# JoelTankard/web-rwkv-gguf

Measured on AMD Instinct MI355X. Metric: tokens/sec RWKV-7 1.5B Q4_K_M decode @1 GPU; achieved HBM GB/s vs roofline, higher is better.
Workload: dtype f16; 1 GPU; RWKV-7 World 1.5B Q4_K_M (Q4_K matrices, Q6_K head, F16 LoRA) batch=1 greedy decode, fused kernels under hipGraph; decode_engine=on, streams_per_gpu=1, pipelines_per_gpu=1, streams=1, parallelism=single

## Files before the change

web-rwkv-gguf_amd/csrc/wrk_v7.hip:

```cpp
#include "wrk_internal.h"
#include "wrk_v7.h"
#include "wrk_v7_engine.h"

#define LOCK(ctx) std::lock_guard<std::recursive_mutex> _lk((ctx)->mu)

static constexpr float LN_EPS = 1.0e-5f;
static constexpr float GN_EPS = 64.0e-5f;
static constexpr float L2_EPS = 1.0e-12f;

using wrk::mat_job;

int32_t wrk_v7_model::ensure_scratch(uint32_t T, uint32_t NH) {
    if (T <= scratch_tokens && NH <= scratch_headers && scratch) return WRK_OK;
    if (ctx->capturing_here()) return wrk_fail(ctx, WRK_E_ARG, "scratch must be sized before capture");
    const uint32_t nt = T > scratch_tokens ? T : scratch_tokens;
    const uint32_t nh = NH > scratch_headers ? NH : scratch_headers;
    WRK_HIP(ctx, hipStreamSynchronize(ctx->stream));
    drop_graphs();
    if (scratch) hipFree(scratch);
    scratch = nullptr;
    const size_t D = d.num_emb, F = d.num_hidden, V = d.num_vocab;
    size_t off = 0;
    auto take = [&](size_t bytes) { size_t o = off; off += wrk_up256(bytes); return o; };
    const size_t esz = act_dtype == WRK_F32 ? 4 : 2;
// ... 449 lines not shown
                     const uint32_t* cursors, uint32_t T, const uint32_t* headers, uint32_t NH, const uint32_t* targets, float* logprob,
                     uint32_t* rank, uint32_t mode) {
    return v7_job(ctx, m, st, {tokens, emb_rows, cursors, T, headers, NH, nullptr, nullptr, true, targets, logprob, rank}, mode);
}

int32_t wrk_v7_model_set_frame_dtype(wrk_ctx* ctx, wrk_v7_model* m, uint32_t dtype) {
    if (!ctx || !m) return WRK_E_ARG;
    LOCK(ctx);
    WRK_ARG(ctx, dtype == WRK_F16 || dtype == WRK_F32, "frame dtype must be WRK_F16 or WRK_F32");
    WRK_ARG(ctx, !ctx->capturing_here(), "cannot change the frame inside a capture");
    if (dtype == m->act_dtype) return WRK_OK;
    WRK_HIP(ctx, hipSetDevice(ctx->device));
    WRK_HIP(ctx, hipStreamSynchronize(ctx->stream));
    m->drop_graphs();
    if (m->scratch) hipFree(m->scratch);
    m->scratch = nullptr;
    m->scratch_tokens = m->scratch_headers = 0;
    m->act_dtype = dtype;
    for (hipStream_t ls : m->lane_streams) WRK_HIP(ctx, hipStreamSynchronize(ls));
    std::vector<wrk_v7_model*> old_lanes;
    old_lanes.swap(m->lanes);
    for (wrk_v7_model* lane : old_lanes) wrk_v7_model_destroy(lane);
    return WRK_OK;
}

int32_t wrk_v7_model_engine_status(wrk_ctx* ctx, wrk_v7_model* m, char* why, size_t capacity) {
    if (!ctx || !m) return WRK_E_ARG;
    LOCK(ctx);
    WRK_HIP(ctx, hipSetDevice(ctx->device));
    WRK_ARG(ctx, !ctx->capturing_here(), "not inside a capture");
    const int32_t rc = m->ensure_engine();
    if (rc != WRK_OK) return rc;
    if (why && capacity) {
        const std::string& w = m->engine ? std::string() : (m->engine_tried ? m->engine_why : std::string("disabled (WRK_ENGINE=0 or f32 frames)"));
        snprintf(why, capacity, "%s", w.c_str());
    }
    return m->engine ? 1 : 0;
}

int32_t wrk_v7_infer_layer(wrk_ctx* ctx, wrk_v7_model* m, wrk_v7_state* st, uint32_t layer, const void* x, const void* v_first,
                           const uint32_t* cursors, uint32_t T, uint32_t mode) {
    if (!ctx || !m || !st || !x || !cursors) return WRK_E_ARG;
    LOCK(ctx);
    WRK_HIP(ctx, hipSetDevice(ctx->device));
    WRK_ARG(ctx, !ctx->capturing_here(), "wrk_v7_infer_layer cannot be captured");
    WRK_ARG(ctx, layer < m->d.num_layer, "layer %u out of range", layer);
    WRK_ARG(ctx, T >= 1, "no tokens");
    WRK_ARG(ctx, layer == 0 || v_first, "layers above 0 read the layer-0 value (att_v0)");
    WRK_ARG(ctx, st->num_emb == m->d.num_emb && st->num_layer == m->d.num_layer, "state does not belong to this model");
    wrk_job_shape sh;
    int32_t rc = wrk_job_check(ctx, st, cursors, T, nullptr, 0, nullptr, 0, &sh);
    if (rc == WRK_OK) rc = m->ensure_scratch(T, 1);
    if (rc == WRK_OK && T == 1 && mode == 1) rc = m->ensure_engine();
    if (rc != WRK_OK) return rc;
    const size_t esz = m->act_dtype == WRK_F32 ? 4 : 2;
    rc = wrk_buf_write_raw(ctx, m->s.cursors, cursors, (size_t)T * 4);
    if (rc == WRK_OK) rc = wrk_buf_write_raw(ctx, m->s.x, x, (size_t)T * m->d.num_emb * esz);
    if (rc == WRK_OK && v_first) rc = wrk_buf_write_raw(ctx, m->s.att_v0, v_first, (size_t)T * m->d.num_emb * esz);
    if (rc != WRK_OK) return rc;
    m->layer_begin = layer; m->layer_end = layer + 1; m->skip_embed = true;
    m->wkv_nseq = sh.nseq;
    { const char* ei = getenv("WRK_ENGINE_INSPECT"); m->engine_skip_once = !(ei && ei[0] == '1'); }
    if (mode == 1 && sh.one_token_each && sh.nseq == T && m->act_dtype == WRK_F16) rc = m->enqueue_fused_decode(st, T, 0, true, false, false, false, cursors[0] & 0xff, sh.contiguous);
    else rc = m->enqueue_ops(st, T, 0, true, mode == 1);
    m->layer_begin = 0; m->layer_end = 0xffffffffu; m->skip_embed = false; m->engine_skip_once = false;
    if (rc != WRK_OK) return rc;
    WRK_LAUNCH_CHECK(ctx);
// ... 147 lines not shown
```

web-rwkv-gguf_amd/csrc/wrk_v7_engine.h:

```cpp
#pragma once
#include <stdint.h>

#include "wrk_internal.h"

namespace wrk {

constexpr int ENG_K1_JOBS = 7;
constexpr uint32_t ENG_NO_HEAD = 0xffffffffu;

struct EngJob {
    uint32_t rows, row_bytes, f16;
    uint32_t act, mix;
    uint32_t wg0, nwg, rows_per_wg;
    uint32_t gbase;
    uint32_t headed;
};

struct EngShape {
    uint32_t D, F, H, nwg;
    uint32_t rw, ra, rg, rv;
    uint32_t rb_d, rb_f;
    uint32_t rb_w2, rb_a2, rb_g2, rb_v2;
    EngJob k1[ENG_K1_JOBS];
    uint32_t k3_rpw, k5_rpw, k6_rpw;
// ... 2 lines not shown
    float ln_eps, gn_eps, l2_eps;
    uint32_t layer_begin, layer_end, rescale;
    uint32_t batch, state_rows;
    uint32_t x_from_granules;
};

struct EngLayer {
    const uint8_t *w_r, *w_k, *w_v, *w1, *a1, *g1, *v1;
    const uint8_t *w2, *a2, *g2, *v2;
    const uint8_t *w_o, *ffn_k, *ffn_v;
};
enum { ENG_V_LN1W, ENG_V_LN1B, ENG_V_LN2W, ENG_V_LN2B, ENG_V_MIX0, ENG_V_W0 = ENG_V_MIX0 + 6, ENG_V_A0, ENG_V_V0, ENG_V_RK, ENG_V_KK, ENG_V_KA,
       ENG_V_GNW, ENG_V_GNB, ENG_V_FFNXK, ENG_NV };
enum { ENG_S_O = ENG_K1_JOBS, ENG_S_FK, ENG_S_FV, ENG_NS = 16 };

struct EngArgs {
    EngShape S;
    const EngLayer* layers;
    const void* vecs;
    const float* scal;
    unsigned long long* gran;
    const void* x_in;
    const uint32_t* x_row;
    void* x_out;
    void* v_first;
    float* state;
    uint32_t num_batch;
    uint32_t* fail;
    unsigned long long* stamps;
    uint32_t stamp_layer;
};
constexpr int ENG_STAMPS = 32;

}

struct wrk_v7_model;
struct wrk_v7_state;
struct wrk_v7_engine;
int32_t wrk_v7_engine_create(wrk_v7_model* m, wrk_v7_engine** out);
void wrk_v7_engine_destroy(wrk_v7_engine* e);
int32_t wrk_v7_engine_enqueue(wrk_v7_engine* e, hipStream_t q, wrk_v7_state* st, uint32_t batch, uint32_t l0, uint32_t l1, const void* x_in,
                              void* x_out, void* v_first, const uint32_t* token = nullptr);
bool wrk_v7_engine_has_table(const wrk_v7_engine* e);
int32_t wrk_v7_engine_check(wrk_v7_engine* e);
void wrk_v7_engine_report(wrk_v7_engine* e);
```

web-rwkv-gguf_amd/csrc/wrk_v7_engine.hip:

```cpp
#include "wrk_device.h"
#include "wrk_v7.h"
#include "wrk_dmv_body.h"
#include "wrk_v7_engine.h"
#include "wrk_lora_dev.h"

#include <algorithm>
#include <string>

namespace wrk {

#define ENG_LDS __attribute__((address_space(3)))
typedef ENG_LDS unsigned char lds_u8;

#define ENG_BAR() asm volatile("s_waitcnt lgkmcnt(0)\n\ts_barrier" ::: "memory")

constexpr uint32_t ENG_SPIN_MAX = 1u << 21;

__device__ __forceinline__ uint32_t eng_tag(uint32_t layer, uint32_t stage) { return layer * 8u + stage + 1u; }

__device__ __forceinline__ void eng_store_granule(unsigned long long* g, uint32_t tag, uint32_t payload) {
    __hip_atomic_store(g, ((unsigned long long)tag << 32) | payload, __ATOMIC_RELAXED, __HIP_MEMORY_SCOPE_AGENT);
}
__device__ __forceinline__ uint32_t pack_h2(float a, float b) {
    const f16x2 h = {(f16)a, (f16)b};
// ... 137 lines not shown
}

struct EngFin {
    uint32_t act;
    float scale;
    const ENG_LDS f16* res;
    float post;
};
__device__ __forceinline__ float eng_finish(const EngFin& f, uint32_t row, float v) {
    float o = act_apply(f.act, v * f.scale);
    if (f.res) o = r16(o) + (float)f.res[row];
    return o;
}

template <int KIND, bool R16, int XI, int RB, class GIDX>
__device__ __forceinline__ void eng_rows(const lds_u8* slot, uint32_t row_bytes, uint32_t K, const ENG_LDS f16* xs, uint32_t row0, uint32_t r_begin,
                                         uint32_t r_end, const EngFin& fin, ENG_LDS uint32_t* pub, unsigned long long* gran, uint32_t tag, GIDX gidx,
                                         uint32_t lane) {
    if (r_begin >= r_end) return;
    const uint32_t kpad = (K + 15u) & ~15u;
    const uint32_t nch = num_chunks<KIND>(K, kpad);
    XRegs x[1][XI];
#pragma unroll
    for (int ci = 0; ci < XI; ++ci) {
        const uint32_t c = lane + 64u * ci;
        x[0][ci] = lds_x<KIND>(xs, min(c, nch - 1));
        if (c >= nch) {
            const f16x8 z = {0, 0, 0, 0, 0, 0, 0, 0};
            x[0][ci].v[0] = x[0][ci].v[1] = x[0][ci].v[2] = x[0][ci].v[3] = z;
        }
        x_sums<KIND>(x[0][ci]);
    }
    static_assert(RB == 2 || RB == 4, "rows per batch");
    for (uint32_t ri = r_begin; ri < r_end; ri += RB) {
        Raw raw[RB][XI];
#pragma unroll
        for (int rb = 0; rb < RB; ++rb) {
            const lds_u8* rowp = slot + (size_t)min(ri + rb, r_end - 1) * row_bytes;
#pragma unroll
            for (int ci = 0; ci < XI; ++ci) raw[rb][ci] = lds_raw<KIND>(rowp, K, min(lane + 64u * ci, nch - 1));
        }
        float v[4] = {0.0f, 0.0f, 0.0f, 0.0f};
#pragma unroll
        for (int rb = 0; rb < RB; ++rb) {
            float acc[1] = {0.0f};
#pragma unroll
            for (int ci = 0; ci < XI; ++ci) dot_raw_tokens<KIND, R16, 1, XI>(raw[rb][ci], min(lane + 64u * ci, nch - 1), x, ci, acc);
            v[rb] = wave_sum(acc[0]);
        }
        if (lane < RB / 2) {
            const uint32_t ra = ri + 2 * lane;
            if (ra < r_end) {
                const float o0 = eng_finish(fin, row0 + ra, lane ? v[2] : v[0]) * fin.post;
                const float o1 = eng_finish(fin, row0 + ra + 1, lane ? v[3] : v[1]) * fin.post;
                if (pub) pub[ra >> 1] = pack_h2(o0, o1);
                else eng_store_granule(gran + gidx(row0 + ra), tag, pack_h2(o0, o1));
            }
        }
    }
}

template <class GIDX>
__device__ __forceinline__ void eng_publish(const ENG_LDS uint32_t* pub, uint32_t nrows, uint32_t row0, unsigned long long* gran, uint32_t tag, GIDX gidx,
                                            uint32_t lane) {
    for (uint32_t i = lane; 2 * i < nrows; i += 64) eng_store_granule(gran + gidx(row0 + 2 * i), tag, pub[i]);
}

template <int VPT>
__device__ __forceinline__ void eng_ln_mix(bool active, const ENG_LDS f16* xraw, ENG_LDS f16* xs, ENG_LDS f16* ln_out, ENG_LDS float* red, uint32_t K, float eps,
                                           const f16x8 (&wv)[VPT], const f16x8 (&bv)[VPT], const f16x8 (&mv)[VPT], const f32x4 (&pv)[VPT][2],
                                           uint32_t tid, uint32_t lane, uint32_t wave) {
    const uint32_t nvec = K >> 3;
    f16x8 xv[VPT];
    float c0 = 0.0f;
    if (active) {
#pragma unroll
        for (int v = 0; v < VPT; ++v) xv[v] = *(const ENG_LDS f16x8*)(xraw + min(tid + 256u * v, nvec - 1) * 8);
        c0 = (float)xraw[0];
        float s1 = 0.0f, s2 = 0.0f;
#pragma unroll
        for (int v = 0; v < VPT; ++v)
            if (tid + 256u * v < nvec)
#pragma unroll
                for (int e = 0; e < 8; ++e) { const float dl = (float)xv[v][e] - c0; s1 += dl; s2 = __builtin_fmaf(dl, dl, s2); }
        s1 = wave_sum(s1);
        s2 = wave_sum(s2);
        if (lane == 0) { red[wave] = s1; red[4 + wave] = s2; }
    }
    ENG_BAR();
    if (active) {
        const float a1 = (red[0] + red[1]) + (red[2] + red[3]);
        const float a2 = (red[4] + red[5]) + (red[6] + red[7]);
        const float md = a1 / (float)K;
        const float mean = c0 + md;
        const float dev = 1.0f / sqrtf(fmaxf(a2 / (float)K - md * md, 0.0f) + eps);
#pragma unroll
        for (int v = 0; v < VPT; ++v) {
            const uint32_t i = tid + 256u * v;
            if (i >= nvec) continue;
            f16x8 yv, o;
#pragma unroll
            for (int e = 0; e < 8; ++e) {
                yv[e] = (f16)__builtin_fmaf(((float)xv[v][e] - mean) * dev, (float)wv[v][e], (float)bv[v][e]);
                o[e] = (f16)wgsl_mix((float)yv[e], pv[v][e >> 2][e & 3], (float)mv[v][e]);
            }
            *(ENG_LDS f16x8*)(xs + i * 8) = o;
            *(ENG_LDS f16x8*)(ln_out + i * 8) = yv;
        }
    }
    ENG_BAR();
}

constexpr int ENG_K2_BARRIERS = 6;
template <int XD, bool R16, int QK, int NCW>
__global__ void __launch_bounds__((NCW + 2) * 64) v7_engine_kernel(const EngArgs A, const uint32_t* __restrict__ wg_head) {
    extern __shared__ __attribute__((aligned(16))) unsigned char eng_smem_generic[];
    lds_u8* smem = (lds_u8*)eng_smem_generic;
    const EngShape& S = A.S;
    const uint32_t tid_all = threadIdx.x;
    const uint32_t wave = (uint32_t)__builtin_amdgcn_readfirstlane((int)(tid_all >> 6));
    const uint32_t wg = blockIdx.x;
    const uint32_t D = S.D, F = S.F;
    const uint32_t head = wg_head[2 * wg], k1r = wg_head[2 * wg + 1];
    const bool is_head = head != ENG_NO_HEAD;
    ENG_LDS uint32_t* abort_flag = (ENG_LDS uint32_t*)(smem + S.lds_misc + 1008);
    ENG_LDS float* red = (ENG_LDS float*)(smem + S.lds_misc);
    ENG_LDS float* part = (ENG_LDS float*)(smem + S.lds_misc + 64);
    ENG_LDS uint32_t* pub = (ENG_LDS uint32_t*)(smem + S.lds_misc + 64);
    ENG_LDS f16* xraw0 = (ENG_LDS f16*)(smem + S.lds_xraw0);
    ENG_LDS f16* xraw1 = (ENG_LDS f16*)(smem + S.lds_xraw1);
    ENG_LDS f16* xs = (ENG_LDS f16*)(smem + S.lds_xs);
    ENG_LDS f16* lnbuf = (ENG_LDS f16*)(smem + S.lds_ln);
    ENG_LDS f16* auxbuf = (ENG_LDS f16*)(smem + S.lds_xs + D * 2u);
    const uint32_t naux = S.rw + S.ra + S.rg + S.rv;
    ENG_LDS float* k2f = (ENG_LDS float*)(smem + S.lds_xs + D * 2u + ((naux + 192u) * 2u + 15u & ~15u));

    uint32_t j1 = ENG_K1_JOBS;
#pragma unroll
    for (int j = 0; j < ENG_K1_JOBS; ++j)
        if (k1r >= S.k1[j].wg0 && k1r < S.k1[j].wg0 + S.k1[j].nwg) j1 = j;
    const uint32_t k1_row0 = j1 < ENG_K1_JOBS ? (k1r - S.k1[j1].wg0) * S.k1[j1].rows_per_wg : 0u;
    const uint32_t k1_rows = j1 < ENG_K1_JOBS ? min(S.k1[j1].rows_per_wg, S.k1[j1].rows - k1_row0) : 0u;
    const uint32_t k1_rb = j1 < ENG_K1_JOBS ? S.k1[j1].row_bytes : 0u;
    const uint32_t k3_row0 = wg * S.k3_rpw, k3_rows = k3_row0 < D ? min(S.k3_rpw, D - k3_row0) : 0u;
    const uint32_t k5_row0 = wg * S.k5_rpw, k5_rows = k5_row0 < F ? min(S.k5_rpw, F - k5_row0) : 0u;
    const uint32_t k6_row0 = wg * S.k6_rpw, k6_rows = k6_row0 < D ? min(S.k6_rpw, D - k6_row0) : 0u;
    const uint32_t srows = S.state_rows;
    auto layer_state = [&](uint32_t l) { return A.state + ((size_t)l * A.num_batch + S.batch) * srows * D; };
    auto k1_src = [&](const EngLayer& L) -> const uint8_t* {
        const uint8_t* base = j1 == 0 ? L.w_r : j1 == 1 ? L.w_k : j1 == 2 ? L.w_v : j1 == 3 ? L.w1 : j1 == 4 ? L.a1 : j1 == 5 ? L.g1 : L.v1;
        return base + (size_t)k1_row0 * k1_rb;
    };
    auto k1_active = [&](uint32_t l) { return j1 < ENG_K1_JOBS && !(j1 == 6 && l == 0) && k1_rows > 0; };
    ENG_LDS unsigned long long* lds_stamps = (ENG_LDS unsigned long long*)(smem + S.lds_misc + 1024);
#define ENG_STAMP(l, k)                                                                                                  \
    do {                                                                                                                 \
        if (A.stamps && (l) == A.stamp_layer && (tid_all & 63u) == 0) lds_stamps[wave * 24 + (k)] = __builtin_amdgcn_s_memrealtime(); \
    } while (0)
#define ENG_STAMP0(l, k) ENG_STAMP(l, k)
#define ENG_FLUSH(l)                                                                                                     \
    do {                                                                                                                 \
        if (A.stamps && (l) == A.stamp_layer && (tid_all & 63u) < 24u)                                                   \
            A.stamps[((size_t)wg * (NCW + 2) + wave) * 24 + (tid_all & 63u)] = lds_stamps[wave * 24 + (tid_all & 63u)];   \
    } while (0)

    if (A.stamps && tid_all < (NCW + 2) * 24) lds_stamps[tid_all] = 0;
    if (tid_all == 0) *abort_flag = 0;
    ENG_BAR();

    if (wave == NCW + 1) {
        const uint32_t lane = tid_all & 63u;
        uint32_t issued = 0, m1 = 0, m3 = 0, m5 = 0, m6 = 0;
        auto fill1 = [&](uint32_t l) { const EngLayer& L = A.layers[l]; issued += eng_fill(k1_src(L), k1_active(l) ? k1_rows * k1_rb : 0u, smem, S.lds_slot1, lane); m1 = issued; };
        auto fill3 = [&](uint32_t l) { const EngLayer& L = A.layers[l]; issued += eng_fill(L.w_o + (size_t)k3_row0 * S.rb_d, k3_rows * S.rb_d, smem, S.lds_slot3, lane); m3 = issued; };
        auto fill5 = [&](uint32_t l) { const EngLayer& L = A.layers[l]; issued += eng_fill(L.ffn_k + (size_t)k5_row0 * S.rb_d, k5_rows * S.rb_d, smem, S.lds_slot5, lane); m5 = issued; };
        auto fill6 = [&](uint32_t l) { const EngLayer& L = A.layers[l]; issued += eng_fill(L.ffn_v + (size_t)k6_row0 * S.rb_f, k6_rows * S.rb_f, smem, S.lds_slot6, lane); m6 = issued; };
        fill1(S.layer_begin); fill3(S.layer_begin); fill5(S.layer_begin); fill6(S.layer_begin);
        bool p6 = false;
        for (uint32_t l = S.layer_begin; l < S.layer_end; ++l) {
            const bool more = l + 1 < S.layer_end;
            eng_wait_vm(issued - m1);
            ENG_BAR();
            if (*abort_flag) break;
            if (p6) { fill6(l); p6 = false; }
            ENG_BAR(); ENG_BAR(); ENG_BAR();
            ENG_STAMP(l, 0);
            if (more) fill1(l + 1);
            if (is_head) {
                ENG_BAR();
                if (*abort_flag) break;
#pragma unroll
                for (int i = 1; i < ENG_K2_BARRIERS; ++i) ENG_BAR();
            }
            eng_wait_vm(issued - m3);
            ENG_BAR();
            if (*abort_flag) break;
            ENG_BAR();
            eng_wait_vm(issued - m5);
            ENG_BAR();
            if (*abort_flag) break;
            if (more) fill3(l + 1);
            ENG_BAR(); ENG_BAR(); ENG_BAR(); ENG_BAR();
            eng_wait_vm(issued - m6);
            ENG_BAR();
            if (*abort_flag) break;
            if (more) fill5(l + 1);
            ENG_BAR(); ENG_BAR();
            p6 = more;
            ENG_FLUSH(l);
        }
        asm volatile("s_waitcnt vmcnt(0)" ::: "memory");
        return;
    }

    if (wave == NCW) {
        const uint32_t lane = tid_all & 63u;
        for (uint32_t l = S.layer_begin; l < S.layer_end; ++l) {
            bool ok = true;
            if (l == S.layer_begin) eng_copy_in(A.x_row ? (const void*)((const f16*)A.x_in + (size_t)A.x_row[0] * D) : A.x_in, D >> 3, (ENG_LDS u32x4*)xraw0, lane);
            else ok = eng_gather(A.gran + S.g_x, D >> 2, eng_tag(l - 1, 4), (ENG_LDS uint32_t*)xraw0, lane);
            if (!ok && lane == 0) { *abort_flag = 1; atomicOr(A.fail, 1u); }
            ENG_STAMP(l, 0);
            ENG_BAR();
            if (*abort_flag) break;
            ENG_BAR(); ENG_BAR(); ENG_BAR();
            if (is_head) {
                ok = eng_gather(A.gran + S.g_k1, (l == 0 ? naux - S.rv : naux) >> 2, eng_tag(l, 0), (ENG_LDS uint32_t*)auxbuf, lane);
                if (ok) ok = eng_gather(A.gran + S.g_k1 + S.g_aux + head * 96u, 48u, eng_tag(l, 0), (ENG_LDS uint32_t*)(auxbuf + naux), lane);
                if (!ok && lane == 0) { *abort_flag = 1; atomicOr(A.fail, 2u); }
                ENG_STAMP(l, 1);
                ENG_BAR();
                if (*abort_flag) break;
#pragma unroll
                for (int i = 1; i < ENG_K2_BARRIERS; ++i) ENG_BAR();
            }
            ok = eng_gather(A.gran + S.g_o, D >> 2, eng_tag(l, 1), (ENG_LDS uint32_t*)xs, lane);
            if (!ok && lane == 0) { *abort_flag = 1; atomicOr(A.fail, 4u); }
            ENG_STAMP(l, 2);
            ENG_BAR();
            if (*abort_flag) break;
            ENG_BAR();
            ok = eng_gather(A.gran + S.g_x1, D >> 2, eng_tag(l, 2), (ENG_LDS uint32_t*)xraw1, lane);
            if (!ok && lane == 0) { *abort_flag = 1; atomicOr(A.fail, 8u); }
            ENG_STAMP(l, 3);
            ENG_BAR();
            if (*abort_flag) break;
            ENG_BAR(); ENG_BAR(); ENG_BAR(); ENG_BAR();
            ENG_BAR();
            if (*abort_flag) break;
            ENG_BAR(); ENG_BAR();
            ENG_FLUSH(l);
        }
        return;
    }

    constexpr int VPT = XD;
    constexpr int S64 = 64;
    constexpr int MAXU = (16 + NCW - 1) / NCW;
    const uint32_t nvec = D >> 3;
    const float eps = S.ln_eps;
    const bool ln_wave = wave < 4;
    auto wave_rows = [&](uint32_t nrows, uint32_t& b, uint32_t& e) {
        const uint32_t q = 2u * (((nrows + 1u) / 2u + NCW - 1u) / NCW);
        b = min(wave * q, nrows);
        e = min(b + q, nrows);
    };
    const uint32_t c0 = is_head ? head * S64 : 0u;
    float vfirst_keep = 0.0f;
    if (is_head && S.layer_begin > 0 && wave == 0) vfirst_keep = (float)((const f16*)A.v_first)[c0 + (tid_all & 63u)];

    unsigned long long clk0 = 0, rt0 = 0;
    if (A.stamps && wg == 0 && tid_all == 0) { clk0 = __builtin_amdgcn_s_memtime(); rt0 = __builtin_amdgcn_s_memrealtime(); }
    for (uint32_t l = S.layer_begin; l < S.layer_end; ++l) {
        uint32_t tid = tid_all;
        asm volatile("" : "+v"(tid));
        const uint32_t lane = tid & 63u;
        float* lst = layer_state(l);
        const bool layer0 = l == 0;
        const f16* lv_base = (const f16*)A.vecs + (size_t)l * ENG_NV * D;
        auto lvec = [&](uint32_t idx) { return lv_base + (size_t)idx * D; };
        const float* scl = A.scal + (size_t)l * ENG_NS;
        const float sc_k1 = scl[j1 < ENG_K1_JOBS ? j1 : 0u], sc_o = scl[ENG_S_O], sc_fk = scl[ENG_S_FK], sc_fv = scl[ENG_S_FV];

        f16x8 wv[VPT], bv[VPT], mv[VPT];
        f32x4 pv[VPT][2];
        if (ln_wave) {
            const f16* mixp = lvec(ENG_V_MIX0 + (j1 < ENG_K1_JOBS ? S.k1[j1].mix : 0u));
#pragma unroll
            for (int v = 0; v < VPT; ++v) {
                const uint32_t i = min(tid + 256u * v, nvec - 1);
                wv[v] = *(const f16x8*)(lvec(ENG_V_LN1W) + i * 8);
                bv[v] = *(const f16x8*)(lvec(ENG_V_LN1B) + i * 8);
                mv[v] = *(const f16x8*)(mixp + i * 8);
                pv[v][0] = *(const f32x4*)(lst + i * 8);
                pv[v][1] = *(const f32x4*)(lst + i * 8 + 4);
            }
        }

        auto request_k5 = [&]() {
            if (ln_wave) {
                float* rowf = lst + (size_t)(srows - 1) * D;
    #pragma unroll
                for (int v = 0; v < VPT; ++v) {
                    const uint32_t i = min(tid + 256u * v, nvec - 1);
                    wv[v] = *(const f16x8*)(lvec(ENG_V_LN2W) + i * 8);
                    bv[v] = *(const f16x8*)(lvec(ENG_V_LN2B) + i * 8);
                    mv[v] = *(const f16x8*)(lvec(ENG_V_FFNXK) + i * 8);
                    pv[v][0] = *(const f32x4*)(rowf + i * 8);
                    pv[v][1] = *(const f32x4*)(rowf + i * 8 + 4);
                }
            }
        };
        if (!is_head) {
            ENG_BAR();
            if (*abort_flag) break;
            ENG_STAMP0(l, 1);
            eng_ln_mix<VPT>(ln_wave, xraw0, xs, lnbuf, red, D, eps, wv, bv, mv, pv, tid, lane, wave);
            ENG_STAMP0(l, 2);
            if (k1_active(l)) {
                const EngJob& J = S.k1[j1];
                uint32_t rb, re;
                wave_rows(k1_rows, rb, re);
                const EngFin fin{J.act, sc_k1, nullptr, 1.0f};
                const lds_u8* slot = smem + S.lds_slot1;
                ENG_LDS uint32_t* nopub = nullptr;
                if (J.f16) {
                    const uint32_t gb = S.g_k1 + J.gbase;
                    eng_rows<WRK_MAT_F16, false, 4 * XD, 2>(slot, k1_rb, D, xs, k1_row0, rb, re, fin, nopub, A.gran, eng_tag(l, 0),
                                                            [&](uint32_t r) { return gb + (r >> 1); }, lane);
                } else {
                    const uint32_t gb = S.g_k1 + S.g_aux + J.gbase * 32u;
                    eng_rows<QK, R16, XD, 4>(slot, k1_rb, D, xs, k1_row0, rb, re, fin, nopub, A.gran, eng_tag(l, 0),
                                             [&](uint32_t r) { return gb + (r >> 6) * 96u + ((r & 63u) >> 1); }, lane);
                }
            }
            ENG_STAMP0(l, 3);
            ENG_BAR();
        } else {
            const EngLayer& Lp = A.layers[l];
            const uint8_t* p_m[4] = {Lp.w2, Lp.a2, Lp.g2, layer0 ? Lp.w2 : Lp.v2};
            const uint32_t rbm[4] = {S.rb_w2, S.rb_a2, S.rb_g2, layer0 ? S.rb_w2 : S.rb_v2};
            const uint32_t rkm[4] = {S.rw, S.ra, S.rg, layer0 ? S.rw : S.rv};
            f16x8 lu[MAXU][8];
#pragma unroll
            for (int i = 0; i < MAXU; ++i) {
                const uint32_t u = min(wave + (uint32_t)i * NCW, 15u), mi = u >> 2, bi = u & 3u;
                const f16* rowp = (const f16*)(p_m[mi] + (size_t)(c0 + 16u * bi + (lane >> 2)) * rbm[mi]);
#pragma unroll
                for (int n = 0; n < 8; ++n) lu[i][n] = *(const f16x8*)(rowp + min((lane & 3u) * 8 + 32 * n, rkm[mi] - 8));
            }
            float Sreg[16];
            const uint32_t ci64 = tid & 63u, g4 = tid >> 6;
            float* st = lst + (size_t)D + c0 + ci64;
            if (ln_wave) {
#pragma unroll
// ... 4 lines not shown
                const uint32_t cc = c0 + lane;
                h_w0 = lvec(ENG_V_W0)[cc]; h_a0 = lvec(ENG_V_A0)[cc]; h_kk = lvec(ENG_V_KK)[cc]; h_ka = lvec(ENG_V_KA)[cc]; h_v0 = lvec(ENG_V_V0)[cc];
                h_gnw = lvec(ENG_V_GNW)[cc]; h_gnb = lvec(ENG_V_GNB)[cc]; h_rk = lvec(ENG_V_RK)[cc];
            }
            ENG_BAR();
            if (*abort_flag) break;
            ENG_STAMP0(l, 1);
            eng_ln_mix<VPT>(ln_wave, xraw0, xs, lnbuf, red, D, eps, wv, bv, mv, pv, tid, lane, wave);
            ENG_STAMP0(l, 3);
            ENG_BAR();

            ENG_LDS float* sh_r = k2f; ENG_LDS float* sh_w = k2f + 64; ENG_LDS float* sh_k = k2f + 128; ENG_LDS float* sh_v = k2f + 192;
            ENG_LDS float* sh_a = k2f + 256; ENG_LDS float* sh_b = k2f + 320; ENG_LDS float* sh_g = k2f + 384; ENG_LDS float* sh_kk = k2f + 448;
            ENG_LDS float* sh_red = k2f + 512;
            ENG_LDS float* sh_red2 = k2f + 768;
            ENG_LDS float* sh_d = k2f + 1024;
            ENG_BAR();
            if (*abort_flag) break;
            ENG_STAMP0(l, 4);
            {
                const ENG_LDS f16* auxm[4] = {auxbuf, auxbuf + S.rw, auxbuf + S.rw + S.ra, layer0 ? auxbuf : auxbuf + S.rw + S.ra + S.rg};
#pragma unroll
                for (int i = 0; i < MAXU; ++i) {
                    const uint32_t u = wave + (uint32_t)i * NCW;
                    if (u < 16u) {
                        const uint32_t mi = u >> 2, bi = u & 3u;
                        const float dd = eng_lora_dot<8>(lu[i], auxm[mi], rkm[mi], lane & 3u);
                        if ((lane & 3u) == 0) sh_d[mi * 64 + 16 * bi + (lane >> 2)] = dd;
                    }
                }
            }
            ENG_STAMP0(l, 16);
            ENG_BAR();
            const ENG_LDS f16* hr = auxbuf + naux, *hk = hr + 64, *hv = hr + 128;
            if (wave == 0) {
                const float w0 = (float)h_w0, a0 = (float)h_a0, kkw = (float)h_kk, kaw = (float)h_ka;
                const float kraw = (float)hk[lane], rraw = (float)hr[lane];
                float v = (float)hv[lane];
                const float v0w = layer0 ? 0.0f : (float)h_v0, vfirst = layer0 ? 0.0f : vfirst_keep;
                const float dw = sh_d[lane], da = sh_d[64 + lane], dg = sh_d[128 + lane], dv = layer0 ? 0.0f : sh_d[192 + lane];
                const float w = r16(w0 + r16(dw));
                const float a = r16(act_sigmoid(a0 + r16(da)));
                const float g = r16(dg);
                if (layer0) { vfirst_keep = v; ((f16*)A.v_first)[c0 + lane] = (f16)v; }
                else {
                    const float vv = r16(act_sigmoid(v0w + r16(dv)));
                    v = r16(wgsl_mix(v, vfirst, vv));
                }
                sh_w[lane] = __expf(-0.606531f * act_sigmoid(w));
                sh_g[lane] = g;
                sh_v[lane] = v;
                sh_r[lane] = rraw;
                const float kkv = r16(kkw * kraw);
                sh_k[lane] = r16(kraw * (1.0f + (a - 1.0f) * kaw));
                const float nrm = 1.0f / sqrtf(wave_sum(kkv * kkv) + S.l2_eps);
                const float kkn = r16(kkv * nrm);
                sh_a[lane] = -kkn;
                sh_b[lane] = kkn * a;
                sh_kk[lane] = kkv;
            }
            if (wave == 1) lst[c0 + lane] = (float)lnbuf[c0 + lane];
            ENG_STAMP0(l, 17);
            ENG_BAR();
            if (ln_wave) {
                float sa = 0.0f;
                f32x4 av[4];
// ... 16 lines not shown
                    for (int e = 0; e < 4; ++e) {
                        const int jj = 4 * q + e, j = g4 * 16 + jj;
                        const float sn = Sreg[jj] * wq[e] + kq4[e] * vv + sa * bq[e];
                        st[(size_t)j * D] = sn;
                        y = __builtin_fmaf(rq4[e], sn, y);
                    }
                }
                sh_red2[g4 * 64 + ci64] = y;
            }
            ENG_STAMP0(l, 18);
            ENG_BAR();
            if (wave == 0) {
                float y = r16((sh_red2[lane] + sh_red2[64 + lane]) + (sh_red2[128 + lane] + sh_red2[192 + lane]));
                const float mean = wave_sum(y) * (1.0f / S64);
                const float dl = y - mean;
                const float var = wave_sum(dl * dl) * (1.0f / S64) + S.gn_eps;
                float o = r16(__builtin_fmaf(dl * (1.0f / sqrtf(var)), (float)h_gnw, (float)h_gnb));
                const float xx = wave_sum((float)h_rk * sh_k[lane] * sh_r[lane]);
                o = r16(o + xx * sh_v[lane]);
                o = sh_g[lane] * o;
                const float o_next = __shfl_down(o, 1, WAVE);
                if ((lane & 1u) == 0) eng_store_granule(A.gran + S.g_o + ((c0 + lane) >> 1), eng_tag(l, 1), pack_h2(o, o_next));
            }
            ENG_STAMP0(l, 5);
            ENG_BAR();
        }

        request_k5();
        ENG_BAR();
        if (*abort_flag) break;
        ENG_STAMP0(l, 6);
        {
            uint32_t rb, re;
            wave_rows(k3_rows, rb, re);
            const EngFin fin{WRK_ACT_NONE, sc_o, xraw0, 1.0f};
            const uint32_t gb = S.g_x1;
            ENG_LDS uint32_t* nopub = nullptr;
            eng_rows<QK, R16, XD, 2>(smem + S.lds_slot3, S.rb_d, D, xs, k3_row0, rb, re, fin, nopub, A.gran, eng_tag(l, 2),
                                     [&](uint32_t r) { return gb + (r >> 1); }, lane);
        }
        ENG_STAMP0(l, 7);
        ENG_BAR();

        ENG_BAR();
        if (*abort_flag) break;
        ENG_STAMP0(l, 8);
        eng_ln_mix<VPT>(ln_wave, xraw1, xs, lnbuf, red, D, eps, wv, bv, mv, pv, tid, lane, wave);
        ENG_STAMP0(l, 14);
        {
            uint32_t rb, re;
            wave_rows(k5_rows, rb, re);
            const EngFin fin{WRK_ACT_SQUARED_RELU, sc_fk, nullptr, 1.0f};
            const uint32_t gb = S.g_k;
            eng_rows<QK, R16, XD, 4>(smem + S.lds_slot5, S.rb_d, D, xs, k5_row0, rb, re, fin, pub, A.gran, eng_tag(l, 3), [&](uint32_t r) { return gb + (r >> 1); }, lane);
            ENG_BAR();
            if (wave == 0) eng_publish(pub, k5_rows, k5_row0, A.gran, eng_tag(l, 3), [&](uint32_t r) { return gb + (r >> 1); }, lane);
        }
        ENG_STAMP0(l, 9);
        ENG_BAR();

        {
            constexpr uint32_t NG = NCW / 4;
            const uint32_t kq = wave & 3u, grp = wave >> 2;
            const bool k6_wave = grp < NG;
            const uint32_t rq = (k6_rows + NG - 1) / NG;
            const uint32_t g_b = min(grp * rq, k6_rows), g_e = min(g_b + rq, k6_rows);
            const uint32_t kpad = (F + 15u) & ~15u;
            const uint32_t nch = num_chunks<QK>(F, kpad);
            const uint32_t cbase = lane + 64u * kq;
            XRegs x[1][XD];
            bool swept = true;
#pragma unroll
            for (int ci = 0; ci < XD; ++ci) {
                const uint32_t c = cbase + 256u * ci;
                x[0][ci].s[0] = x[0][ci].s[1] = 0.0f;
                const f16x8 z = {0, 0, 0, 0, 0, 0, 0, 0};
                x[0][ci].v[0] = x[0][ci].v[1] = x[0][ci].v[2] = x[0][ci].v[3] = z;
                if (k6_wave && g_b < g_e && swept) swept = eng_sweep_x<QK>(A.gran + S.g_k, min(c, nch - 1), eng_tag(l, 3), x[0][ci]);
                if (c >= nch) x[0][ci].v[0] = x[0][ci].v[1] = x[0][ci].v[2] = x[0][ci].v[3] = z;
                x_sums<QK>(x[0][ci]);
            }
            if (!swept && lane == 0) { *abort_flag = 1; atomicOr(A.fail, 16u); }
            ENG_STAMP0(l, 10);
            ENG_BAR();
// ... 250 lines not shown
    }
    {
        hipFuncAttributes fa{};
        const int waves = e->ncw + 2, per_simd = (waves + 3) / 4;
        if (hipFuncGetAttributes(&fa, fn) == hipSuccess && fa.numRegs > 0) {
            const int alloc = (fa.numRegs + 7) / 8 * 8;
            if (per_simd * alloc > 512 || fa.maxThreadsPerBlock < waves * 64 || (size_t)fa.sharedSizeBytes + S.lds_total > 160 * 1024) {
                const int regs = fa.numRegs;
                wrk_v7_engine_destroy(e);
                return wrk_fail(ctx, WRK_E_UNSUPPORTED, "decode engine: a workgroup of %d waves x %d registers + %u bytes of LDS does not fit a CU", waves, regs,
                                S.lds_total);
            }
        }
        (void)hipGetLastError();
    }
    {
        const char* te = getenv("WRK_ENGINE_TABLE");
        if (!(te && te[0] == '0') && m->emb && m->ln0_w && m->ln0_b) {
            const size_t bytes = (size_t)d.num_vocab * D * 2;
            if (hipMalloc(&e->emb_ln, bytes) == hipSuccess) {
                LnMixParams P{};
                P.src = (const f16*)m->emb->ptr; P.ln_w = (const f16*)m->ln0_w->ptr; P.ln_b = (const f16*)m->ln0_b->ptr; P.eps = 1.0e-5f;
                P.d = D; P.nmix = 0; P.ln_out = (f16*)e->emb_ln;
                if (ln_mix(ctx->stream, P, d.num_vocab) != 0 || hipStreamSynchronize(ctx->stream) != hipSuccess) { hipFree(e->emb_ln); e->emb_ln = nullptr; }
            } else e->emb_ln = nullptr;
            (void)hipGetLastError();
        }
    }
    *out = e;
    return WRK_OK;
}

bool wrk_v7_engine_has_table(const wrk_v7_engine* e) { return e && e->emb_ln; }

void wrk_v7_engine_destroy(wrk_v7_engine* e) {
    if (!e) return;
    if (e->emb_ln) hipFree(e->emb_ln);
    if (e->layers) hipFree(e->layers);
    if (e->vecs) hipFree(e->vecs);
    if (e->scal) hipFree(e->scal);
    if (e->wg_head) hipFree(e->wg_head);
    if (e->gran) hipFree(e->gran);
    if (e->fail) hipFree(e->fail);
    if (e->stamps) hipFree(e->stamps);
    delete e;
}

int32_t wrk_v7_engine_enqueue(wrk_v7_engine* e, hipStream_t q, wrk_v7_state* st, uint32_t batch, uint32_t l0, uint32_t l1, const void* x_in, void* x_out,
                              void* v_first, const uint32_t* token) {
    using namespace wrk;
    wrk_ctx* ctx = e->m->ctx;
    EngArgs A{};
    A.S = e->S;
    A.S.layer_begin = l0; A.S.layer_end = l1; A.S.batch = batch;
    A.layers = e->layers; A.vecs = e->vecs; A.scal = e->scal; A.gran = e->gran; A.x_in = x_in; A.x_out = x_out; A.v_first = v_first;
    if (token && e->emb_ln && l0 == 0) { A.x_in = e->emb_ln; A.x_row = token; }
    A.state = st->data; A.num_batch = st->num_batch; A.fail = e->fail; A.stamps = e->stamps; A.stamp_layer = std::min(5u, l1 - 1);
    WRK_HIP(ctx, hipMemsetAsync(e->gran, 0, (size_t)e->S.g_total * 8, q));
    const dim3 grid(e->S.nwg), block((e->ncw + 2) * 64);
    hipLaunchKernelGGL(eng_kernel(e->xd, e->r16, e->ncw), grid, block, e->S.lds_total, q, A, (const uint32_t*)e->wg_head);
    WRK_LAUNCH_CHECK(ctx);
    return WRK_OK;
}

int32_t wrk_v7_engine_check(wrk_v7_engine* e) {
    if (!e) return WRK_OK;
    wrk_ctx* ctx = e->m->ctx;
    uint32_t f = 0;
    WRK_HIP(ctx, hipMemcpy(&f, e->fail, 4, hipMemcpyDeviceToHost));
    if (f) {
        hipMemset(e->fail, 0, 4);
        return wrk_fail(ctx, WRK_E_HIP, "decode engine: a hand-off wait gave up (stage mask 0x%x): workgroups not co-resident or a producer died", f);
    }
    return WRK_OK;
}

void wrk_v7_engine_report(wrk_v7_engine* e) {
    using namespace wrk;
    if (!e || !e->stamps) return;
    const uint32_t NWG = e->S.nwg, NW = (uint32_t)e->ncw + 2;
    std::vector<unsigned long long> h((size_t)NWG * NW * 24);
    if (hipMemcpy(h.data(), e->stamps, h.size() * 8, hipMemcpyDeviceToHost) != hipSuccess) return;
    unsigned long long t0 = ~0ull;
    for (auto v : h) if (v && v < t0) t0 = v;
    auto col = [&](int wave, uint32_t k, const char* label) {
        std::vector<double> v;
        for (uint32_t w = 0; w < NWG; ++w) {
            unsigned long long x = 0;
            if (wave >= 0) x = h[((size_t)w * NW + wave) * 24 + k];
            else for (int cw = 0; cw < e->ncw; ++cw) x = std::max(x, h[((size_t)w * NW + cw) * 24 + k]);
            if (x) v.push_back((double)(x - t0) * 0.01);
        }
        if (v.empty()) return;
        std::sort(v.begin(), v.end());
        fprintf(stderr, "  %-62s %4zu WGs  first %7.2f  median %7.2f  last %7.2f us\n", label, v.size(), v.front(), v[v.size() / 2], v.back());
    };
    {
        unsigned long long tail[2] = {0, 0};
        if (hipMemcpy(tail, e->stamps + (size_t)NWG * 16 * 24, 16, hipMemcpyDeviceToHost) == hipSuccess && tail[1])
            fprintf(stderr, "[WRK_TIMING] decode engine: shader clock over the last launch %.0f MHz (%llu cycles in %.1f us)\n",
                    (double)tail[0] / ((double)tail[1] * 0.01), tail[0], (double)tail[1] * 0.01);
    }
    const int G = e->ncw, Ld = e->ncw + 1;
    fprintf(stderr, "[WRK_TIMING] decode engine (%d compute waves), one layer of the last token; us since the layer's first stamp\n", e->ncw);
    col(G, 0, "gather: layer input complete");
    col(0, 1, "K1 start (input + weights in LDS), wave 0");
    col(0, 2, "K1 LN + shift done, wave 0");
    col(0, 3, "K1 rows published, wave 0");
    col(-1, 3, "K1 rows published, slowest wave");
    col(G, 1, "gather (heads): K1 outputs complete");
    col(0, 4, "K2 start");
    col(-1, 16, "K2 LoRA dots done, slowest wave");
    col(0, 17, "K2 per-channel stage done");
    col(-1, 18, "K2 state updated, slowest wave");
    col(0, 5, "K2 published");
    col(G, 2, "gather: head outputs complete");
    col(0, 6, "K3 start");
    col(-1, 7, "K3 published, slowest wave");
    col(G, 3, "gather: x1 complete");
    col(0, 8, "K5 start");
    col(0, 14, "K5 LN + shift done, wave 0");
    col(0, 9, "K5 published, wave 0");
    col(-1, 9, "K5 published, slowest wave");
    col(0, 10, "K6 own quarter of the ffn vector swept, wave 0");
    col(-1, 10, "K6 swept, slowest wave");
    col(0, 11, "K6 start");
    col(-1, 12, "K6 partial sums done, slowest wave");
    col(0, 13, "K6 published");
    col(Ld, 0, "loader: K1 slot free, next layer's fill issued");
}
```

Measured before the change: 1674 tokens/s.

## Split head gather into two stages and balance row pairs across SIMDs

The head workgroups' gather now runs in two phases. LoRA intermediates are gathered first and signalled through a separate abort flag, so K2's LoRA dots can start before the per-head K1 outputs arrive, and the second gather overlaps that work. Row-pair assignment per compute wave now comes from a constexpr schedule that spreads leftover pairs evenly across SIMDs instead of giving each wave a fixed chunk, with static_asserts checking coverage. The row loop also skips dot products for a partial trailing batch. Barrier counts are centralized as constants, and the timing report gains head and non-head breakdowns.

```diff
diff --git a/web-rwkv-gguf_amd/csrc/wrk_v7.hip b/web-rwkv-gguf_amd/csrc/wrk_v7.hip
--- a/web-rwkv-gguf_amd/csrc/wrk_v7.hip
+++ b/web-rwkv-gguf_amd/csrc/wrk_v7.hip
@@ -505,7 +505,8 @@
     const int32_t rc = m->ensure_engine();
     if (rc != WRK_OK) return rc;
     if (why && capacity) {
-        const std::string& w = m->engine ? std::string() : (m->engine_tried ? m->engine_why : std::string("disabled (WRK_ENGINE=0 or f32 frames)"));
+        const std::string w = m->engine ? std::to_string(wrk_v7_engine_waves(m->engine)) + " compute waves"
+                                        : (m->engine_tried ? m->engine_why : std::string("disabled (WRK_ENGINE=0 or f32 frames)"));
         snprintf(why, capacity, "%s", w.c_str());
     }
     return m->engine ? 1 : 0;
diff --git a/web-rwkv-gguf_amd/csrc/wrk_v7_engine.h b/web-rwkv-gguf_amd/csrc/wrk_v7_engine.h
--- a/web-rwkv-gguf_amd/csrc/wrk_v7_engine.h
+++ b/web-rwkv-gguf_amd/csrc/wrk_v7_engine.h
@@ -58,6 +58,44 @@
 };
 constexpr int ENG_STAMPS = 32;
 
+constexpr __host__ __device__ uint32_t eng_wave_pairs(uint32_t pairs, uint32_t ncw, uint32_t wave) {
+    const uint32_t simd_rank = (wave + 4u - (ncw + 2u) % 4u) % 4u;
+    return pairs / ncw + ((wave / 4u) * 4u + simd_rank < pairs % ncw ? 1u : 0u);
+}
+constexpr __host__ __device__ uint32_t eng_wave_first_pair(uint32_t pairs, uint32_t ncw, uint32_t wave) {
+    const uint32_t extra = pairs % ncw, g4 = (wave / 4u) * 4u;
+    uint32_t first = wave * (pairs / ncw) + (extra < g4 ? extra : g4);
+    for (uint32_t w = g4; w < wave; ++w) first += eng_wave_pairs(pairs, ncw, w) - pairs / ncw;
+    return first;
+}
+constexpr __host__ __device__ void eng_wave_rows(uint32_t nrows, uint32_t ncw, uint32_t wave, uint32_t& begin, uint32_t& end) {
+    const uint32_t pairs = (nrows + 1u) / 2u;
+    const uint32_t first = eng_wave_first_pair(pairs, ncw, wave), last = first + eng_wave_pairs(pairs, ncw, wave);
+    begin = 2u * first < nrows ? 2u * first : nrows;
+    end = 2u * last < nrows ? 2u * last : nrows;
+}
+constexpr bool eng_wave_rows_ok(uint32_t ncw) {
+    for (uint32_t nrows = 0; nrows <= 128; nrows += 2) {
+        const uint32_t pairs = nrows / 2, most = (pairs + ncw - 1) / ncw;
+        uint32_t next = 0, simd[4] = {0, 0, 0, 0};
+        for (uint32_t w = 0; w < ncw; ++w) {
+            uint32_t b = 0, e = 0;
+            eng_wave_rows(nrows, ncw, w, b, e);
+            if (b != next || e < b || (b & 1u) || (e & 1u) || (e - b) / 2 > most || (e - b) / 2 < pairs / ncw) return false;
+            simd[w % 4] += (e - b) / 2 - pairs / ncw;
+            next = e;
+        }
+        if (next != nrows) return false;
+        const uint32_t s0 = (ncw + 2) % 4;
+        for (uint32_t i = 0; i + 1 < 4; ++i) {
+            const uint32_t a = simd[(s0 + i) % 4], c = simd[(s0 + i + 1) % 4];
+            if (c > a || simd[s0] - simd[(s0 + 3) % 4] > 1) return false;
+        }
+    }
+    return true;
+}
+static_assert(eng_wave_rows_ok(8) && eng_wave_rows_ok(14), "a row pair without exactly one owner wave, or an uneven schedule");
+
 }
 
 struct wrk_v7_model;
@@ -68,5 +106,6 @@
 int32_t wrk_v7_engine_enqueue(wrk_v7_engine* e, hipStream_t q, wrk_v7_state* st, uint32_t batch, uint32_t l0, uint32_t l1, const void* x_in,
                               void* x_out, void* v_first, const uint32_t* token = nullptr);
 bool wrk_v7_engine_has_table(const wrk_v7_engine* e);
+int wrk_v7_engine_waves(const wrk_v7_engine* e);
 int32_t wrk_v7_engine_check(wrk_v7_engine* e);
 void wrk_v7_engine_report(wrk_v7_engine* e);
diff --git a/web-rwkv-gguf_amd/csrc/wrk_v7_engine.hip b/web-rwkv-gguf_amd/csrc/wrk_v7_engine.hip
--- a/web-rwkv-gguf_amd/csrc/wrk_v7_engine.hip
+++ b/web-rwkv-gguf_amd/csrc/wrk_v7_engine.hip
@@ -193,7 +193,9 @@
         x_sums<KIND>(x[0][ci]);
     }
     static_assert(RB == 2 || RB == 4, "rows per batch");
+    constexpr bool PAD = XI > 1;
     for (uint32_t ri = r_begin; ri < r_end; ri += RB) {
+        const bool whole = PAD || RB == 2 || ri + RB <= r_end;
         Raw raw[RB][XI];
 #pragma unroll
         for (int rb = 0; rb < RB; ++rb) {
@@ -203,12 +205,13 @@
         }
         float v[4] = {0.0f, 0.0f, 0.0f, 0.0f};
 #pragma unroll
-        for (int rb = 0; rb < RB; ++rb) {
-            float acc[1] = {0.0f};
-#pragma unroll
-            for (int ci = 0; ci < XI; ++ci) dot_raw_tokens<KIND, R16, 1, XI>(raw[rb][ci], min(lane + 64u * ci, nch - 1), x, ci, acc);
-            v[rb] = wave_sum(acc[0]);
-        }
+        for (int rb = 0; rb < RB; ++rb)
+            if (rb < 2 || whole) {
+                float acc[1] = {0.0f};
+#pragma unroll
+                for (int ci = 0; ci < XI; ++ci) dot_raw_tokens<KIND, R16, 1, XI>(raw[rb][ci], min(lane + 64u * ci, nch - 1), x, ci, acc);
+                v[rb] = wave_sum(acc[0]);
+            }
         if (lane < RB / 2) {
             const uint32_t ra = ri + 2 * lane;
             if (ra < r_end) {
@@ -272,7 +275,18 @@
     ENG_BAR();
 }
 
+constexpr int ENG_LN_BARRIERS = 2;
+constexpr int ENG_K1_BARRIERS = 2 + ENG_LN_BARRIERS;
 constexpr int ENG_K2_BARRIERS = 6;
+constexpr int ENG_K2_CHECKED = 2;
+constexpr int ENG_K3_BARRIERS = 2;
+constexpr int ENG_K5_BARRIERS = 3 + ENG_LN_BARRIERS;
+constexpr int ENG_K6_BARRIERS = 3;
+template <int N>
+__device__ __forceinline__ void eng_replay() {
+#pragma unroll
+    for (int i = 0; i < N; ++i) ENG_BAR();
+}
 template <int XD, bool R16, int QK, int NCW>
 __global__ void __launch_bounds__((NCW + 2) * 64) v7_engine_kernel(const EngArgs A, const uint32_t* __restrict__ wg_head) {
     extern __shared__ __attribute__((aligned(16))) unsigned char eng_smem_generic[];
@@ -326,7 +340,7 @@
     } while (0)
 
     if (A.stamps && tid_all < (NCW + 2) * 24) lds_stamps[tid_all] = 0;
-    if (tid_all == 0) *abort_flag = 0;
+    if (tid_all == 0) { abort_flag[0] = 0; abort_flag[1] = 0; }
     ENG_BAR();
 
     if (wave == NCW + 1) {
@@ -344,29 +358,30 @@
             ENG_BAR();
             if (*abort_flag) break;
             if (p6) { fill6(l); p6 = false; }
-            ENG_BAR(); ENG_BAR(); ENG_BAR();
+            eng_replay<ENG_K1_BARRIERS - 1>();
             ENG_STAMP(l, 0);
             if (more) fill1(l + 1);
             if (is_head) {
                 ENG_BAR();
                 if (*abort_flag) break;
-#pragma unroll
-                for (int i = 1; i < ENG_K2_BARRIERS; ++i) ENG_BAR();
+                ENG_BAR();
+                if (abort_flag[1]) break;
+                eng_replay<ENG_K2_BARRIERS - ENG_K2_CHECKED>();
             }
             eng_wait_vm(issued - m3);
             ENG_BAR();
             if (*abort_flag) break;
-            ENG_BAR();
+            eng_replay<ENG_K3_BARRIERS - 1>();
             eng_wait_vm(issued - m5);
             ENG_BAR();
             if (*abort_flag) break;
             if (more) fill3(l + 1);
-            ENG_BAR(); ENG_BAR(); ENG_BAR(); ENG_BAR();
+            eng_replay<ENG_K5_BARRIERS - 1>();
             eng_wait_vm(issued - m6);
             ENG_BAR();
             if (*abort_flag) break;
             if (more) fill5(l + 1);
-            ENG_BAR(); ENG_BAR();
+            eng_replay<ENG_K6_BARRIERS - 1>();
             p6 = more;
             ENG_FLUSH(l);
         }
@@ -384,32 +399,35 @@
             ENG_STAMP(l, 0);
             ENG_BAR();
             if (*abort_flag) break;
-            ENG_BAR(); ENG_BAR(); ENG_BAR();
+            eng_replay<ENG_K1_BARRIERS - 1>();
             if (is_head) {
                 ok = eng_gather(A.gran + S.g_k1, (l == 0 ? naux - S.rv : naux) >> 2, eng_tag(l, 0), (ENG_LDS uint32_t*)auxbuf, lane);
-                if (ok) ok = eng_gather(A.gran + S.g_k1 + S.g_aux + head * 96u, 48u, eng_tag(l, 0), (ENG_LDS uint32_t*)(auxbuf + naux), lane);
                 if (!ok && lane == 0) { *abort_flag = 1; atomicOr(A.fail, 2u); }
+                ENG_STAMP(l, 4);
+                ENG_BAR();
+                if (*abort_flag) break;
+                ok = eng_gather(A.gran + S.g_k1 + S.g_aux + head * 96u, 48u, eng_tag(l, 0), (ENG_LDS uint32_t*)(auxbuf + naux), lane);
+                if (!ok && lane == 0) { abort_flag[1] = 1; atomicOr(A.fail, 2u); }
                 ENG_STAMP(l, 1);
                 ENG_BAR();
-                if (*abort_flag) break;
-#pragma unroll
-                for (int i = 1; i < ENG_K2_BARRIERS; ++i) ENG_BAR();
+                if (abort_flag[1]) break;
+                eng_replay<ENG_K2_BARRIERS - ENG_K2_CHECKED>();
             }
             ok = eng_gather(A.gran + S.g_o, D >> 2, eng_tag(l, 1), (ENG_LDS uint32_t*)xs, lane);
             if (!ok && lane == 0) { *abort_flag = 1; atomicOr(A.fail, 4u); }
             ENG_STAMP(l, 2);
             ENG_BAR();
             if (*abort_flag) break;
-            ENG_BAR();
+            eng_replay<ENG_K3_BARRIERS - 1>();
             ok = eng_gather(A.gran + S.g_x1, D >> 2, eng_tag(l, 2), (ENG_LDS uint32_t*)xraw1, lane);
             if (!ok && lane == 0) { *abort_flag = 1; atomicOr(A.fail, 8u); }
             ENG_STAMP(l, 3);
             ENG_BAR();
             if (*abort_flag) break;
-            ENG_BAR(); ENG_BAR(); ENG_BAR(); ENG_BAR();
-            ENG_BAR();
-            if (*abort_flag) break;
-            ENG_BAR(); ENG_BAR();
+            eng_replay<ENG_K5_BARRIERS - 1>();
+            ENG_BAR();
+            if (*abort_flag) break;
+            eng_replay<ENG_K6_BARRIERS - 1>();
             ENG_FLUSH(l);
         }
         return;
@@ -421,11 +439,6 @@
     const uint32_t nvec = D >> 3;
     const float eps = S.ln_eps;
     const bool ln_wave = wave < 4;
-    auto wave_rows = [&](uint32_t nrows, uint32_t& b, uint32_t& e) {
-        const uint32_t q = 2u * (((nrows + 1u) / 2u + NCW - 1u) / NCW);
-        b = min(wave * q, nrows);
-        e = min(b + q, nrows);
-    };
     const uint32_t c0 = is_head ? head * S64 : 0u;
     float vfirst_keep = 0.0f;
     if (is_head && S.layer_begin > 0 && wave == 0) vfirst_keep = (float)((const f16*)A.v_first)[c0 + (tid_all & 63u)];
@@ -481,7 +494,7 @@
             if (k1_active(l)) {
                 const EngJob& J = S.k1[j1];
                 uint32_t rb, re;
-                wave_rows(k1_rows, rb, re);
+                eng_wave_rows(k1_rows, NCW, wave, rb, re);
                 const EngFin fin{J.act, sc_k1, nullptr, 1.0f};
                 const lds_u8* slot = smem + S.lds_slot1;
                 ENG_LDS uint32_t* nopub = nullptr;
@@ -552,6 +565,7 @@
             }
             ENG_STAMP0(l, 16);
             ENG_BAR();
+            if (abort_flag[1]) break;
             const ENG_LDS f16* hr = auxbuf + naux, *hk = hr + 64, *hv = hr + 128;
             if (wave == 0) {
                 const float w0 = (float)h_w0, a0 = (float)h_a0, kkw = (float)h_kk, kaw = (float)h_ka;
@@ -634,7 +648,7 @@
         ENG_STAMP0(l, 6);
         {
             uint32_t rb, re;
-            wave_rows(k3_rows, rb, re);
+            eng_wave_rows(k3_rows, NCW, wave, rb, re);
             const EngFin fin{WRK_ACT_NONE, sc_o, xraw0, 1.0f};
             const uint32_t gb = S.g_x1;
             ENG_LDS uint32_t* nopub = nullptr;
@@ -651,7 +665,7 @@
         ENG_STAMP0(l, 14);
         {
             uint32_t rb, re;
-            wave_rows(k5_rows, rb, re);
+            eng_wave_rows(k5_rows, NCW, wave, rb, re);
             const EngFin fin{WRK_ACT_SQUARED_RELU, sc_fk, nullptr, 1.0f};
             const uint32_t gb = S.g_k;
             eng_rows<QK, R16, XD, 4>(smem + S.lds_slot5, S.rb_d, D, xs, k5_row0, rb, re, fin, pub, A.gran, eng_tag(l, 3), [&](uint32_t r) { return gb + (r >> 1); }, lane);
@@ -968,6 +982,7 @@
 }
 
 bool wrk_v7_engine_has_table(const wrk_v7_engine* e) { return e && e->emb_ln; }
+int wrk_v7_engine_waves(const wrk_v7_engine* e) { return e ? e->ncw : 0; }
 
 void wrk_v7_engine_destroy(wrk_v7_engine* e) {
     if (!e) return;
@@ -1019,9 +1034,12 @@
     if (hipMemcpy(h.data(), e->stamps, h.size() * 8, hipMemcpyDeviceToHost) != hipSuccess) return;
     unsigned long long t0 = ~0ull;
     for (auto v : h) if (v && v < t0) t0 = v;
-    auto col = [&](int wave, uint32_t k, const char* label) {
+    std::vector<char> is_head(NWG, 0);
+    for (uint32_t hd = 0; hd < e->S.H; ++hd) is_head[(size_t)hd * NWG / e->S.H] = 1;
+    auto col = [&](int wave, uint32_t k, const char* label, int cls = -1) {
         std::vector<double> v;
         for (uint32_t w = 0; w < NWG; ++w) {
+            if (cls >= 0 && is_head[w] != cls) continue;
             unsigned long long x = 0;
             if (wave >= 0) x = h[((size_t)w * NW + wave) * 24 + k];
             else for (int cw = 0; cw < e->ncw; ++cw) x = std::max(x, h[((size_t)w * NW + cw) * 24 + k]);
@@ -1039,11 +1057,15 @@
     }
     const int G = e->ncw, Ld = e->ncw + 1;
     fprintf(stderr, "[WRK_TIMING] decode engine (%d compute waves), one layer of the last token; us since the layer's first stamp\n", e->ncw);
-    col(G, 0, "gather: layer input complete");
-    col(0, 1, "K1 start (input + weights in LDS), wave 0");
+    col(G, 0, "gather: layer input complete, workgroups without a head", 0);
+    col(G, 0, "gather: layer input complete, head workgroups", 1);
+    col(0, 1, "K1 start (input + weights in LDS), wave 0, no head", 0);
+    col(0, 1, "K1 start (input in LDS), wave 0, head workgroups", 1);
     col(0, 2, "K1 LN + shift done, wave 0");
-    col(0, 3, "K1 rows published, wave 0");
-    col(-1, 3, "K1 rows published, slowest wave");
+    col(0, 3, "K1 rows published, wave 0, no head", 0);
+    col(-1, 3, "K1 rows published, slowest wave, no head", 0);
+    col(-1, 3, "K1 LN + shift done, slowest wave, head workgroups", 1);
+    col(G, 4, "gather (heads): LoRA intermediates complete");
     col(G, 1, "gather (heads): K1 outputs complete");
     col(0, 4, "K2 start");
     col(-1, 16, "K2 LoRA dots done, slowest wave");
```

New measurement: 1726 tokens/s, median of 6. 3.1% higher.
